# flexcompute/tidy3d

Hardware: AMD Instinct MI355X
Metric: Mcells/s on 512^3 Yee grid (higher is better)
Workload: dtype f32; 1 GPU; v0: vacuum, PEC walls, curl stencil only; 512^3 Yee cells, Ez point dipole (GaussianPulse 200 THz), random +-1e-3 initial fields; parallelism=z-slab x1, bytes_per_cell_step=72

## Files before the change

include/fdtd_hip.h:

```cpp
#ifndef FDTD_HIP_H
#define FDTD_HIP_H

#include <stddef.h>
#include <stdint.h>

#ifdef __cplusplus
extern "C" {
#endif

typedef struct FdtdSolver FdtdSolver;

enum { FDTD_BC_PEC = 0, FDTD_BC_PMC = 1, FDTD_BC_PERIODIC = 2, FDTD_BC_NEIGHBOR = 3 };
enum { FDTD_MON_TIME = 0, FDTD_MON_DFT = 1, FDTD_MON_FLUX_TIME = 2 ,
       FDTD_MON_TIME_SPARSE = 3 ,
       FDTD_MON_DFT_SPARSE = 4 ,
       FDTD_MON_DFT_LATTICE = 5  };
enum { FDTD_VARIANT_AUTO = 0, FDTD_VARIANT_SIMPLE = 1, FDTD_VARIANT_ZMARCH = 2, FDTD_VARIANT_FUSED = 3 };
enum { FDTD_FLAG_TIME_KERNELS = 1 };

typedef struct FdtdConfig {
  int32_t nx, ny, nz;
  int32_t bc[6];
  int32_t device;
  int32_t variant;
// ... 173 lines not shown
       FDTD_OPT_EDGE_ZCHUNK = 14,
       FDTD_OPT_GRAPH = 15,
       FDTD_OPT_TWOSTEP = 16,
       FDTD_OPT_SHELL_PAIRS = 17,
       FDTD_OPT_STRIP = 18,
       FDTD_OPT_SHELL2 = 19,
       FDTD_OPT_SHELL2_SHAPE = 20,
       FDTD_OPT_DEBUG_SYNC = 21,
       FDTD_OPT_TILE_SPLIT = 22,
       FDTD_OPT_DISP = 23,
       FDTD_OPT_SRC_PAGED = 25,
       FDTD_OPT_WHATIF = 24,
       FDTD_OPT_SLAB_BOXES_FIRST = 26,
       FDTD_OPT_SEAM_DEFER = 27,
       FDTD_OPT_AXIS_SHIFT = 28,
       FDTD_OPT_LDS_PAD = 10  };
int fdtd_set_option(FdtdSolver* h, int key, int value);
int fdtd_get_seam_stats(FdtdSolver* h, FdtdSeamStats* out);
int fdtd_reset(FdtdSolver* h);

#define FDTD_SWEEP_WORD(lb, opt, w) (((int64_t)(w) << 48) | ((int64_t)(lb) << 32) | (int64_t)(opt))
#define FDTD_SWEEP_WORD_OPT(word) ((int)((word) & 0xffffffff))
#define FDTD_SWEEP_WORD_LB(word) ((int)(((word) >> 32) & 0xffff))
#define FDTD_SWEEP_WORD_W(word) ((int)(((word) >> 48) & 0xff))
int fdtd_get_sweep_words(FdtdSolver* h, int64_t* out, int cap);
int fdtd_sweep_table(int64_t* out, int cap);

#ifdef __cplusplus
}
#endif
#endif
```

tidy3d_amd/csrc/fdtd_capi.hip:

```cpp
#include <hip/hip_runtime.h>
#include <rccl/rccl.h>

#include <array>
#include <cmath>
#include <cstdarg>
#include <cstdio>
#include <cstdlib>
#include <cstring>
#include <deque>
#include <map>
#include <string>
#include <utility>
#include <algorithm>
#include <vector>

#include "../../include/fdtd_hip.h"
#include "fdtd_kernels.hpp"
#include "fdtd_fused2.hpp"
#include "fdtd_strip.hpp"
#include "fdtd_shell2_host.hpp"
#include "fdtd_aniso.hpp"
#include "fdtd_modulation.hpp"
#include "fdtd_conformal.hpp"
#include "fdtd_near_field.hpp"
// ... 179 lines not shown
  std::string err;
  std::vector<DevBuf> bufs;
  float* fbase[6] = {};
  FieldP f{};
  float* fbase2[6] = {};
  FieldP f2{};
  float* fbase3[6] = {};
  FieldP f3{};
  float* step_base[2] = {};
  size_t field_bytes = 0;
  float *ip[3] = {}, *idl[3] = {};
  uint32_t* mat4 = nullptr;
  uint32_t* mat4b = nullptr;
  uint32_t* roww = nullptr;
  std::vector<uint32_t> roww_host;
  struct TileClasses { int W, zc; ClipP box; int nbx, nby, nbz; unsigned char* dev; long long n_bg, n_all; bool disp, src; };
  std::vector<TileClasses> tile_cls;
  int tile_split = -1;
  float2* lut = nullptr;
  int n_media = 0;
  float ca1 = 1.f, cb1 = 0.f;
  std::vector<float> cb_host;
  PmlAxisDev pml[3];
  float *damp_fb[3] = {}, *damp_fc[3] = {};
  int damp_lo[3] = {0, 0, 0}, damp_hi[3] = {0, 0, 0};
  bool has_damp = false;
  std::vector<AdeGroup> ade;
  Disp disp;
  SrcPaged spg;
  std::map<std::array<int, 6>, int> box_paged;
  int spg_on = -1;
  int whatif = 0;
// ... 787 lines not shown
    }
    tb.dump_floats = off;
    if (!boxes.empty()) {
      std::vector<int> ds((size_t)g.nz + 2, 0), dl;
      for (int k = 0; k <= g.nz; ++k) { ds[(size_t)k] = (int)dl.size(); if (k < g.nz) for (int b : per_plane[(size_t)k]) dl.push_back(b); }
      ds[(size_t)g.nz + 1] = (int)dl.size();
      if (dl.empty()) dl.push_back(0);
      if (dev_upload(h, &tb.dstart, (const int*)ds.data(), ds.size()) || dev_upload(h, &tb.dlist, (const int*)dl.data(), dl.size()) ||
          dev_upload(h, &tb.dboxes, (const DumpBox*)boxes.data(), boxes.size())) return nullptr;
    }
  }
  h->f2_tables.push_back(tb);
  return &h->f2_tables.back();
}

const FdtdSolver::TileClasses* tile_classes(FdtdSolver* h, int W, int zc, const ClipP& box, int nbx, int nby, int nbz, bool disp = false, bool src = false) {
  const bool mats = h->mat4 && !h->roww_host.empty();
  if ((!mats && !src) || h->tile_split == 0) return nullptr;
  for (const auto& t : h->tile_cls)
    if (t.W == W && t.zc == zc && t.nbx == nbx && t.nby == nby && t.nbz == nbz && t.box.j0 == box.j0 && t.box.j1 == box.j1 &&
        t.box.k0 == box.k0 && t.box.k1 == box.k1 && t.disp == disp && t.src == src) return &t;
  const GridP& g = h->g;
  const int R = W - 3, nbx_all = (g.nx + 255) / 256;
  std::vector<unsigned char> cls((size_t)nbx * nby * nbz, 0);
  long long n_bg = 0;
  for (int tz = 0; tz < nbz; ++tz)
    for (int tx = 0; tx < nbx; ++tx)
      for (int ty = 0; ty < nby; ++ty) {
        const int k0 = box.k0 + tz * zc, k1 = std::min(k0 + zc, box.k1);
        const int j0 = box.j0 + ty * R;
        unsigned char c = 0;
        for (int k = std::max(k0 - 1, 0); mats && k <= std::min(k1, g.nz - 1) && !c; ++k)
          for (int j = std::max(j0 - 2, 0); j <= std::min(j0 + R, g.ny - 1); ++j)
            if (h->roww_host[((size_t)k * g.ny + j) * nbx_all + tx] != kBgWord) { c = 1; break; }
        if (disp && c)
          for (int k = std::max(k0 - 1, 0); k <= std::min(k1, g.nz - 1) && c < 2; ++k)
            for (int j = std::max(j0 - 2, 0); j <= std::min(j0 + R, g.ny - 1); ++j)
              if (h->disp.dseg_host[((size_t)k * g.ny + j) * nbx_all + tx] >= 0) { c = 2; break; }
        n_bg += !c;
        if (src) {
          bool found = false;
          for (int k = std::max(k0 - 1, 0); k <= std::min(k1, g.nz - 1) && !found; ++k)
            for (int j = std::max(j0 - 2, 0); j <= std::min(j0 + R, g.ny - 1); ++j)
              if (h->spg.sseg_host[((size_t)k * g.ny + j) * nbx_all + tx] >= 0) { found = true; break; }
          if (found) c |= 4;
        }
        cls[((size_t)tz * nbx + tx) * nby + ty] = c;
      }
  FdtdSolver::TileClasses e{W, zc, box, nbx, nby, nbz, nullptr, n_bg, (long long)cls.size(), disp, src};
  if (dev_upload(h, &e.dev, (const unsigned char*)cls.data(), cls.size())) return nullptr;
  h->tile_cls.push_back(e);
  return &h->tile_cls.back();
}

void flush_seams(FdtdSolver* h, hipStream_t st);
int launch_fused2(FdtdSolver* h, long long n, hipStream_t st, const F2Table* tb, bool* sources2_done, bool* damp2_done = nullptr,
                  const ClipP* clip = nullptr, bool use_disp = false, bool e2_clip = false, const SrcP& sr = SrcP{}, bool defer_ok = false) {
  const bool inject = tb->with_sources;
  const GridP& g = h->g;
  if (use_disp && !h->mat4) return fail(h, "launch_fused2: dispersive cells in a pair without the materials grid");
  if (ensure_second_set(h)) return -1;
  int W = 16, zc = 32;
  const ClipP box = clip ? *clip : ClipP{0, g.nx, 0, g.ny, 0, g.nz};
  fused2_shape(h, &W, &zc, (clip && h->comm) ? clip : nullptr);
  if (clip && !h->comm && h->twostep_zc <= 0 && (long long)g.nx * g.ny * g.nz < (1LL << 28)) zc = std::min(zc, 16);
  zc = std::max(2, std::min(zc, box.k1 - box.k0));
  h->twostep_w_used = W; h->twostep_zc_used = zc;
// ... 60 lines not shown
      S.sseg_host.assign(nseg, -1);
      SrcT tab{};
      if (dev_upload(h, &S.sseg, (const int*)S.sseg_host.data(), nseg) || dev_upload(h, &S.tab, &tab, 1)) return -1;
    }
    if (S.sseg && S.state != 1) { sr_used.sseg = S.sseg; sr_used.t = S.tab; }
  }
  const int wv = h->whatif == 19 ? 9 : ((h->whatif >= 1 && h->whatif <= 15 && h->whatif != 9) ? h->whatif : 0);
  const auto word = [&](bool rep) {
    return fused2_opt(h->mem_hints != 0, h->mat4 != nullptr, !(tb->mons.empty() && (!tb->with_sources || h->src_h_nodes == 0) && !tb->dstart),
                      clip != nullptr, damp, use_disp, sr_used.sseg != nullptr, wv, rep, W);
  };
  const bool rep_capable = n_seams > 0 && !clip && (W == 16 || h->seam_defer == 2) && fused2_rep_word(word(false));
  const int opt = word(rep_capable && (h->seam_pending || h->whatif == 17));
  const auto no_sweep = [&] { return fail(h, "launch_fused2: no instantiation of the sweep for opt 0x%x, %d waves", opt, W); };
  if (!fused2_instantiated(fused2_lb(W, opt), opt)) return no_sweep();
  if (sr.sseg) { *sources2_done = true; h->spg.pairs++; }
  float* const rep_arr = h->seam_buf ? h->seam_buf + seam_scratch_floats(g, nbx) : nullptr;
  if (h->seam_pending && !rep_capable) flush_seams(h, st);
  h->seam_pending = false;
  bool defer = defer_ok && rep_capable && h->seam_defer != 0 && h->whatif == 0;
  if (defer) {
    bool e_post = false;
    for (const PointSrc& s : h->psrc) e_post = e_post || (s.n_e && n + 1 < s.n_steps);
    if ((e_post && !*sources2_done) || (h->has_damp && !dmp.e2)) defer = false;
  }
  const int blocks = remap ? ((total + 7) / 8) * 8 : total;
  const FdtdSolver::TileClasses* tc = tile_classes(h, W, zc, box, nbx, nby, nbz, use_disp, sr_used.sseg != nullptr);
  const bool split = tc && (use_disp || sr_used.sseg || (tc->n_bg > 0 && (h->tile_split == 1 || 8 * tc->n_bg >= tc->n_all)));
  const bool launched = launch_fused2_step(Fused2Launch{st, W, opt, blocks, g, h->f, h->f2, sp, mp, zc, nbx, nby, nbz, remap, inj, h->seam_buf, dmp, box,
                                                        TileClassP{split ? tc->dev : nullptr}, dp, sr_used});
  time_end(h, st);
  if (!launched) return no_sweep();
  {
    const int64_t word = FDTD_SWEEP_WORD(fused2_lb(W, opt), opt, W);
    if (std::find(h->sweep_words.begin(), h->sweep_words.end(), word) == h->sweep_words.end()) h->sweep_words.push_back(word);
  }
  if (n_seams > 0 && !(rep_capable && (h->whatif == 16 || h->whatif == 17))) {
    time_begin(h, 4, st);
    launch_seams(st, g, h->f2, sp, mp, h->seam_buf, n_seams, dmp, box, inj, sr, (defer || (h->whatif == 18 && rep_capable)) ? rep_arr : nullptr);
    time_end(h, st);
  }
  if (use_disp) h->disp.pairs++;
  if (!clip) swap_sets(h);
  if (defer) { h->seam_pending = true; h->seam_deferred_pairs++; }
  return 0;
// ... 1506 lines not shown
    return fail(nullptr, "fdtd_create: slab of %d x %d x %d cells exceeds the 2^32 cell index range", cfg->nx, cfg->ny, cfg->nz);
  for (int a = 0; a < 3; ++a) {
    const bool p0 = cfg->bc[2 * a] == FDTD_BC_PERIODIC, p1 = cfg->bc[2 * a + 1] == FDTD_BC_PERIODIC;
    if (p0 != p1 && a < 2) return fail(nullptr, "fdtd_create: periodic boundary must be set on both faces of axis %d", a);
    if (cfg->bc[2 * a + 1] == FDTD_BC_PMC) return fail(nullptr, "fdtd_create: PMC is supported on min faces only");
    if (a < 2 && (cfg->bc[2 * a] == FDTD_BC_NEIGHBOR || cfg->bc[2 * a + 1] == FDTD_BC_NEIGHBOR))
      return fail(nullptr, "fdtd_create: neighbour faces exist only along z");
  }
  int ndev = 0;
  if (hipGetDeviceCount(&ndev) != hipSuccess || ndev < 1) return fail(nullptr, "fdtd_create: no HIP device available");
  if (cfg->device < 0 || cfg->device >= ndev) return fail(nullptr, "fdtd_create: device %d out of range (%d devices)", cfg->device, ndev);
  FdtdSolver* h = new FdtdSolver();
  h->cfg = *cfg;
  h->no_jlo = getenv("FDTD_NO_JLO") != nullptr;
  if (hipSetDevice(cfg->device) != hipSuccess) { delete h; return fail(nullptr, "hipSetDevice(%d) failed", cfg->device); }
  GridP& g = h->g;
  g.nx = cfg->nx; g.ny = cfg->ny; g.nz = cfg->nz;
  g.sxy = (long long)cfg->nx * cfg->ny;
  g.bcx0 = cfg->bc[0]; g.bcx1 = cfg->bc[1]; g.bcy0 = cfg->bc[2]; g.bcy1 = cfg->bc[3];
  g.pec_z0 = cfg->bc[4] == FDTD_BC_PEC;
  g.psi_ghost = cfg->bc[4] == FDTD_BC_NEIGHBOR ? 1 : 0;
  g.ch = cfg->ch;
  h->zchunk = cfg->z_chunk > 0 ? cfg->z_chunk : 2;
  h->zchunk_f = cfg->z_chunk > 0 ? cfg->z_chunk : 16;
  h->user_geometry = cfg->z_chunk > 0;
  h->rows = 4;
  int rc = 0;
  const size_t fcount = (size_t)g.sxy * (g.nz + 2);
  h->field_bytes = fcount * sizeof(float);
  rc = alloc_field_set(h, h->fbase, fcount, 0);
// ... 889 lines not shown
    }
    case FDTD_OPT_PML_SPLIT: h->pml_split = value < 0 ? -1 : (value != 0); return 0;
    case FDTD_OPT_SHELL_PAIRS: h->shell_on = value < 0 ? -1 : value; return 0;
    case FDTD_OPT_STRIP: if (value % 64 < 1 || (value / 64 != 3 && value / 64 != 4)) break; h->strip_zc = value % 64; h->strip_occ = value / 64; return 0;
    case FDTD_OPT_SHELL2: h->shell2_on = value < 0 ? -1 : (value > 3 ? 1 : value); return 0;
    case FDTD_OPT_DEBUG_SYNC: h->debug_sync = value != 0; return 0;
    case FDTD_OPT_TILE_SPLIT: h->tile_split = value < 0 ? -1 : (value != 0); return 0;
    case FDTD_OPT_SRC_PAGED:
      h->spg_on = value < 0 ? -1 : (value != 0);
      if (h->spg.state == -1 && value != 0) h->spg.state = 0;
      return 0;
    case FDTD_OPT_SLAB_BOXES_FIRST: if (value < 0 || value > 3) break; h->slab_boxes_first = value; return 0;
    case FDTD_OPT_WHATIF: if (value < 0 || value > 19) break; h->whatif = value; return 0;
    case FDTD_OPT_SEAM_DEFER: if (value > 2) break; h->seam_defer = value < 0 ? -1 : value; return 0;
    case FDTD_OPT_AXIS_SHIFT: if (value < 0 || value > 2) break; h->axis_shift = value; return 0;
    case FDTD_OPT_DISP:
      if (h->disp.state == 1 && value == 0) break;
      h->disp_on = value < 0 ? -1 : (value != 0);
      if (h->disp.state == -1 && value != 0) h->disp.state = 0;
      return 0;
    case FDTD_OPT_SHELL2_SHAPE: {
      if (value <= 0) { h->shell2_qw = 0; h->shell2_ww = 8; h->shell2_zcw = 0; h->shell2_ws = 6; h->shell2_zcs = 0; return 0; }
      const int qw = value % 128, ww = (value >> 7) % 8 + ((value >> 7) % 8 == 0 ? 8 : 0), zcw = (value >> 10) % 128;
      const int ws = (value >> 17) % 16, zcs = (value >> 21) % 128;
      if ((qw != 0 && qw < 3) || qw > 64 || ws > 8) break;
      h->shell2_qw = qw; h->shell2_ww = ww; h->shell2_zcw = zcw;
      h->shell2_ws = ws > 0 ? ws : 6; h->shell2_zcs = zcs;
      return 0;
    }
    case FDTD_OPT_FUSED_LB: if (value != 0 && value != 256 && value != 512 && value != 1024) break; h->fused_lb = value; return 0;
// ... 27 lines not shown
  out->src_paged_pairs = (int32_t)std::min<long long>(h->spg.pairs, 0x7fffffff);
  out->struct_bytes = (int32_t)sizeof(FdtdStats);
  return 0;
}

int fdtd_get_seam_stats(FdtdSolver* h, FdtdSeamStats* out) {
  if (!h || !out) return -1;
  out->seam_deferred_pairs = h->seam_deferred_pairs;
  out->seam_flushes = h->seam_flushes;
  out->seam_pending = h->seam_pending ? 1 : 0;
  out->reserved = 0;
  out->seam_flush_ms = h->seam_flush_ms;
  return 0;
}

int fdtd_get_sweep_words(FdtdSolver* h, int64_t* out, int cap) {
  if (!h || (cap > 0 && !out)) return -1;
  const int n = (int)h->sweep_words.size();
  for (int i = 0; i < n && i < cap; ++i) out[i] = h->sweep_words[i];
  return n;
}

int fdtd_sweep_table(int64_t* out, int cap) {
  if (cap > 0 && !out) return -1;
  static const int64_t table[] = {
#define FDTD_F2_X(LBV, OV) FDTD_SWEEP_WORD(LBV, OV, 0),
      FDTD_F2_LIST_ALL(FDTD_F2_X)
#undef FDTD_F2_X
  };
  const int n = (int)(sizeof(table) / sizeof(table[0]));
// ... 6 lines not shown
```

tidy3d_amd/csrc/fdtd_fused2.hpp:

```cpp
#pragma once
#include "fdtd_kernels.hpp"

namespace fdtd {

constexpr int kMaxInj = 256;
struct InjP {
  int n;
  const int* start;
  const int4* ent;
  const float* val;
  const float* val2;
  int e2_in_sweep;
  float* cap;
  const int* dstart;
  const int* dlist;
  const struct DumpBox* dboxes;
  float* dump;
};
struct DumpBox {
  int lo0, lo1, lo2, nx, ny, nz;
  int off[6];
};
constexpr int kMaxDumps = 8;
struct DampT {
  const float* fb[3];
  const float* fc[3];
  int e2;
};
struct ClipP { int i0, i1, j0, j1, k0, k1; };
struct TileClassP { const unsigned char* cls; };
struct DispP {
  const int* dseg;
  const float* cs;
  float* e1;
};
struct SrcT {
  const float* e1;
  const float* h2;
  const float* e2;
  int use_h2, use_e2;
  const float* e1b;
  const float* h2b;
  const float* e2b;
};
struct SrcP {
  const int* sseg = nullptr;
  const SrcT* t = nullptr;
};
constexpr int kF2NT = 1;
constexpr int kF2Mat = 2;
constexpr int kF2Mon = 4;
constexpr int kF2Damp = 8;
constexpr int kF2Clip = 16;
constexpr int kF2Disp = 32;
constexpr int kF2Src = 64;
constexpr int kF2WhatifShift = 8, kF2WhatifMask = 15;
constexpr int kF2NoExj = 4096;
constexpr int kF2Rep = 8192;
constexpr int fused2_whatif(int opt) { return (opt >> kF2WhatifShift) & kF2WhatifMask; }
constexpr int fused2_whatif_word(int wv) { return kF2NT | (wv << kF2WhatifShift); }
constexpr bool fused2_rep_word(int opt) { return (opt & ~(kF2NT | kF2Mat | kF2Damp)) == 0; }

constexpr int fused2_opt(bool nt, bool mat, bool mon, bool clip, bool damp, bool disp, bool src, int whatif, bool rep, int W) {
  int opt = (nt ? kF2NT : 0) | (mat ? kF2Mat : 0) | (mon ? kF2Mon : 0) | (clip ? kF2Clip : (damp ? kF2Damp : 0)) |
            (disp ? kF2Disp | kF2NT : 0) | (src ? kF2Src | kF2Mon | kF2NT : 0);
  if (whatif && opt == kF2NT && (W == 16 || whatif == 13 || whatif == 14)) opt = fused2_whatif_word(whatif);
  return opt | (rep ? kF2Rep : 0);
}
constexpr int fused2_lb(int waves, int opt) {
  if ((opt & kF2Rep) || fused2_whatif(opt)) return 1024;
  if (waves <= 8) return 512;
  return (waves <= 12 && !(opt & (kF2Src | kF2Disp))) ? 768 : 1024;
}

#define FDTD_F2_AT512(X, O) X(512, (O))
#define FDTD_F2_AT768(X, O) X(768, (O))
// ... 68 lines not shown
  return fused2_lds_bytes(lb, opt, w) == ((size_t)(fused2_exj(lb, opt) ? 9 : 8) * w * 64 + ((opt & 8) ? 2 * 64 : 0)) * sizeof(float4) + ((opt & 2) ? (size_t)kMaxMedia * sizeof(float2) : 0);
}
#define FDTD_F2_X(LBV, OV) && fused2_lds_pinned(LBV, OV)
static_assert(true FDTD_F2_LIST_ALL(FDTD_F2_X), "fused2_lds_bytes: the LDS of a listed instantiation changed");
#undef FDTD_F2_X
constexpr int kMaxCap = 1024;
constexpr int kSeamArrays = 13;

void launch_inject_values(hipStream_t st, float* val, const float* w_re, const float* w_im, const float2* wave,
                          long long step, int n);
struct Fused2Launch {
  hipStream_t st;
  int waves, opt, grid_blocks;
  GridP g; FieldP a, b; StepP s; MatP m;
  int zchunk, nbx, nby, nbz, xcd_remap;
  InjP inj; float* seam; DampT dmp; ClipP clip; TileClassP tcl; DispP dp; SrcP sr;
};
#define FDTD_F2_ARGS(L) (L).g, (L).a, (L).b, (L).s, (L).m, (L).zchunk, (L).nbx, (L).nby, (L).nbz, (L).xcd_remap, (L).inj, (L).seam, (L).dmp, (L).clip, (L).tcl, (L).dp, (L).sr
#define FDTD_F2_CASE(LBV, OV)                                                                                                      \
  case fused2_key(LBV, OV):                                                                                                        \
    hipLaunchKernelGGL((fused2_step_kernel<LBV, OV>), dim3(L.grid_blocks, 1, 1), dim3(64, L.waves, 1), fused2_lds_bytes(LBV, OV, L.waves), L.st, \
                       FDTD_F2_ARGS(L));                                                                                           \
    return true;
#define FDTD_F2_LAUNCHER(NAME, LIST)                                                                                               \
  bool NAME(const Fused2Launch& L) {                                                                                               \
    switch (fused2_key(fused2_lb(L.waves, L.opt), L.opt)) { LIST(FDTD_F2_CASE) default: return false; }                            \
  }
bool launch_fused2_step(const Fused2Launch& L);
bool launch_fused2_step_src(const Fused2Launch& L);
bool launch_fused2_step_whatif(const Fused2Launch& L);
bool launch_fused2_step_disp(const Fused2Launch& L);
bool launch_fused2_step_clip(const Fused2Launch& L);
void launch_inject_table(hipStream_t st, float* tab, long long stride, long long off, const float* w_re, const float* w_im,
// ... 26 lines not shown
```

tidy3d_amd/csrc/fdtd_kernels2.hpp:

```cpp
#pragma once
#include "fdtd_fused2.hpp"

namespace fdtd {

__global__ __launch_bounds__(256) void pair_record_kernel(PairRecP r, GridP g, FieldP a, FieldP b, const float* cap) {
  const int mi = blockIdx.y / 6, ic = blockIdx.y % 6;
  if (mi >= r.n_mon || ic >= r.nc[mi]) return;
  const BoxP bx = r.box[mi];
  const long long cells = (long long)bx.nx * bx.ny * bx.nz;
  const long long t = (long long)blockIdx.x * blockDim.x + threadIdx.x;
  if (t >= cells) return;
  const int c = r.comp[mi][ic];
  const int lx = (int)(t % bx.nx), ly = (int)((t / bx.nx) % bx.ny), lz = (int)(t / ((long long)bx.nx * bx.ny));
  const long long p = (long long)(bx.lo2 + lz) * g.sxy + (long long)(bx.lo1 + ly) * g.nx + bx.lo0 + lx;
  const long long idx = (long long)ic * cells + t;
  const float* fa = c == 0 ? a.ex : (c == 1 ? a.ey : (c == 2 ? a.ez : (c == 3 ? a.hx : (c == 4 ? a.hy : a.hz))));
  const float* fb = c == 0 ? b.ex : (c == 1 ? b.ey : (c == 2 ? b.ez : (c == 3 ? b.hx : (c == 4 ? b.hy : b.hz))));
  const float mid = cap[r.cap_off[mi] + idx];
  float* on = r.out_n[mi];
  float* om = r.out_m[mi];
  if (c < 3) {
    if (on && !r.pre_done) on[idx] = 1.0f * fa[p];
    if (om) om[idx] = 1.0f * mid;
  } else {
// ... 93 lines not shown
  return v;
}

__device__ __forceinline__ int lane_value(int v, int l) {
#if defined(__HIP_DEVICE_COMPILE__)
  return __builtin_amdgcn_readlane(v, l);
#else
  return __shfl(v, l);
#endif
}

template <int LB, int OPT>
__device__ __forceinline__ void fused2_step_tile(const GridP& g, const FieldP& a, const FieldP& b, const StepP& s, const MatP& m,
                                                 int zchunk, int nbx, int nby, int nbz, const InjP& inj,
                                                 float* __restrict__ seam, const DampT& dmp, const ClipP& clip, int t,
                                                 const DispP& dp, const SrcP& sr) {
  constexpr int V = 4;
  constexpr bool SRC = (OPT & kF2Src) != 0;
  constexpr bool NT = (OPT & kF2NT) != 0, MAT = (OPT & kF2Mat) != 0, MON = (OPT & kF2Mon) != 0;
  constexpr bool DISP = (OPT & kF2Disp) != 0;
  constexpr int WHATIF = fused2_whatif(OPT);
  constexpr int PF = (WHATIF >= 10 && WHATIF <= 12) ? WHATIF : 0;
  constexpr bool EZL = WHATIF == 15;
  constexpr bool EXJ = (WHATIF == 0 && (OPT & kF2NoExj) == 0) || WHATIF == 13 || EZL;
  constexpr bool E1S = PF != 0 || EZL;
  constexpr int XE = E1S ? 6 : 8, XZ = 7;
  [[maybe_unused]] constexpr int NPF = PF == 11 ? 2 : (PF ? 3 : 0);
  constexpr int NXCH = E1S ? 6 : 8;
  static_assert((!PF && !EZL) || (OPT & 0xff & ~kF2NT) == 0, "prefetch instantiations: the vacuum sweep only");
  constexpr bool DAMP = (OPT & kF2Damp) != 0;
  constexpr bool CLIP = (OPT & kF2Clip) != 0;
  constexpr bool REP = (OPT & kF2Rep) != 0;
  static_assert(!REP || (!CLIP && !PF && !EZL && !DISP && !SRC), "deferred seam repair: plain, materials and absorber sweeps of the whole grid");
  const bool per_x = CLIP && g.bcx0 == BC_PERIODIC;
  const int tile_y = t % nby;
  const int tile_x = (t / nby) % nbx;
  const int tile_z = t / (nby * nbx);
  HIP_DYNAMIC_SHARED(float4, xch)
  const int tx = threadIdx.x;
  const int ty = __builtin_amdgcn_readfirstlane((int)threadIdx.y);
  const int W = blockDim.y, R = W - 3;
  const int slot = W * 64;
  const int me = ty * 64 + tx;
  {
    const float4 z4 = {0.f, 0.f, 0.f, 0.f};
#pragma unroll
    for (int q = 0; q < NXCH; ++q) xch[q * slot + me] = z4;
  }
  [[maybe_unused]] float4* xdm = xch + (EXJ ? 9 : 8) * slot;
  [[maybe_unused]] float2* lut_s = reinterpret_cast<float2*>(xdm + (DAMP ? 2 * 64 : 0));
  if constexpr (MAT) {
    for (int q = me; q < m.n_media; q += slot) lut_s[q] = m.lut[q];
  }
  if constexpr (DAMP) {
    if (ty == 0) {
      const int ii = (tile_x * 64 + tx) * V;
      float4 b4 = {1.f, 1.f, 1.f, 1.f}, c4 = {1.f, 1.f, 1.f, 1.f};
      if (ii < g.nx) { b4 = *reinterpret_cast<const float4*>(dmp.fb[0] + ii); c4 = *reinterpret_cast<const float4*>(dmp.fc[0] + ii); }
      xdm[tx] = b4; xdm[64 + tx] = c4;
    }
  }
  __syncthreads();
  const float ca = m.ca1, cb = m.cb1;
  const int k0 = (CLIP ? clip.k0 : 0) + tile_z * zchunk;
  const int k1 = min(k0 + zchunk, CLIP ? clip.k1 : g.nz);
  const int kA = k0 > 0 ? k0 - 1 : 0;
  int j = (CLIP ? clip.j0 : 0) + tile_y * R + ty - 2;
  const bool row_ok = (j >= 0) && (j < g.ny);
  if (!row_ok) {
    if constexpr (WHATIF != 6 && WHATIF != 7 && WHATIF != 8)
      for (int k = kA; k <= k1; ++k) { __syncthreads(); if constexpr (WHATIF != 2) __syncthreads(); }
    return;
  }
  const int i0 = (tile_x * 64 + tx) * V;
  const unsigned ux = (unsigned)i0;
  const unsigned ub = ux * 4u;
  const unsigned ubc = (i0 < g.nx) ? ub : 0u;
  const bool act = (i0 < g.nx);
  const bool do_e1 = ty >= 1;
  const bool do_h2 = ty >= 1 && ty <= W - 2;
// ... 758 lines not shown
    if constexpr (DAMP) { bz_m = bzk; cz_m = czk; }
    if constexpr (MAT) rw_m = rw;
    if constexpr (SRC) ss_m = ss;
    cur ^= 1;
  };
  if constexpr (PF != 0) pf_issue(kA);
  for (int k = kA; k <= k1; k += 2) {
    body(k, LA);
    if (k + 1 <= k1) body(k + 1, LB2);
  }
}

template <int LB, int OPT>
__device__ __forceinline__ void fused2_tile_by_class(const GridP& g, const FieldP& a, const FieldP& b, const StepP& s, const MatP& m,
                                                     int zchunk, int nbx, int nby, int nbz, const InjP& inj, float* __restrict__ seam,
                                                     const DampT& dmp, const ClipP& clip, int t, const DispP& dp, const SrcP& sr, const TileClassP& tcl) {
  if constexpr ((OPT & kF2Mat) != 0) {
    if (tcl.cls) {
      const int cl = tcl.cls[t] & 3;
      if (cl == 0) {
        fused2_step_tile<LB, (OPT & ~(kF2Mat | kF2Disp))>(g, a, b, s, m, zchunk, nbx, nby, nbz, inj, seam, dmp, clip, t, dp, sr);
        return;
      }
      if constexpr ((OPT & kF2Disp) != 0) {
        if (cl == 1) {
          fused2_step_tile<LB, (OPT & ~kF2Disp)>(g, a, b, s, m, zchunk, nbx, nby, nbz, inj, seam, dmp, clip, t, dp, sr);
          return;
        }
      }
    }
  }
  fused2_step_tile<LB, OPT>(g, a, b, s, m, zchunk, nbx, nby, nbz, inj, seam, dmp, clip, t, dp, sr);
}

template <int LB, int OPT>
__global__ __launch_bounds__(LB, (LB == 512 ? 4 : 1)) void fused2_step_kernel(GridP g, FieldP a, FieldP b, StepP s, MatP m,
                                                         int zchunk, int nbx, int nby, int nbz, int xcd_remap,
                                                         InjP inj, float* __restrict__ seam, DampT dmp, ClipP clip, TileClassP tcl, DispP dp, SrcP sr) {
  const int total = nbx * nby * nbz;
  int t = blockIdx.x;
  if (xcd_remap == 1) {
    const int per = (total + 7) >> 3;
    t = (t & 7) * per + (t >> 3);
    if (t >= total) return;
  } else if (xcd_remap > 1) {
    const int G = xcd_remap, full = total / (8 * G) * (8 * G);
    if (t < full) {
      const int x = t & 7, mloc = t >> 3;
      t = ((mloc / G) * 8 + x) * G + mloc % G;
    }
    if (t >= total) return;
  }
  constexpr int OPTK = OPT | (fused2_exj(LB, OPT) ? 0 : kF2NoExj);
  if constexpr ((OPT & kF2Src) != 0) {
    if (tcl.cls && !(tcl.cls[t] & 4)) {
      fused2_tile_by_class<LB, (OPTK & ~kF2Src)>(g, a, b, s, m, zchunk, nbx, nby, nbz, inj, seam, dmp, clip, t, dp, sr, tcl);
      return;
    }
  }
  fused2_tile_by_class<LB, OPTK>(g, a, b, s, m, zchunk, nbx, nby, nbz, inj, seam, dmp, clip, t, dp, sr, tcl);
}

__global__ __launch_bounds__(256) void seam_kernel(GridP g, FieldP b, StepP s, MatP m,
                                                   const float* __restrict__ seam, int n_seams, DampT dmp, ClipP clip, InjP inj, SrcP sr,
                                                   float* __restrict__ rep) {
  const long long t = (long long)blockIdx.x * blockDim.x + threadIdx.x;
  const int nj = clip.j1 - clip.j0;
  const long long per = (long long)nj * (clip.k1 - clip.k0);
  if (t >= per * n_seams) return;
  const int sm = (int)(t / per);
  const int k = clip.k0 + (int)((t % per) / nj), j = clip.j0 + (int)(t % nj);
  const bool wrap = g.bcx0 == BC_PERIODIC && sm == n_seams - 1;
  const int c = wrap ? g.nx : (sm + 1) * 256;
  const int cc = wrap ? 0 : c;
  const bool wl = c - 1 >= clip.i0 && c - 1 < clip.i1, wr = cc >= clip.i0 && cc < clip.i1;
// ... 110 lines not shown
```

tidy3d_amd/lib.py:

```python
from __future__ import annotations

import ctypes as C
import os
from typing import Optional

from .exceptions import SolverLibraryError

_HERE = os.path.dirname(os.path.abspath(__file__))
DEFAULT_LIB = os.path.join(_HERE, "libfdtd_hip.so")



def _prefer_hw_queues() -> None:
    os.environ.setdefault("GPU_MAX_HW_QUEUES", "8")


SYMBOLS = (
    "fdtd_last_error", "fdtd_device_count", "fdtd_create", "fdtd_destroy", "fdtd_set_steps",
    "fdtd_set_media", "fdtd_set_material", "fdtd_set_material16", "fdtd_set_pml", "fdtd_set_absorber", "fdtd_add_ade",
    "fdtd_add_point_source", "fdtd_add_tfsf", "fdtd_add_monitor", "fdtd_get_monitor",
    "fdtd_set_field", "fdtd_get_field", "fdtd_set_shutoff", "fdtd_comm_unique_id",
    "fdtd_comm_init", "fdtd_run", "fdtd_run_bloch", "fdtd_get_stats", "fdtd_reset", "fdtd_set_option",
    "fdtd_far_field", "fdtd_set_mirror_plus", "fdtd_add_aniso", "fdtd_add_aniso_bloch", "fdtd_get_seam_stats",
    "fdtd_get_sweep_words", "fdtd_sweep_table", "fdtd_add_flux_time_monitor", "fdtd_get_monitor_bytes",
    "fdtd_add_field_time_monitor", "fdtd_add_field_dft_monitor", "fdtd_add_lattice_dft_monitor", "fdtd_add_modulation",
    "fdtd_add_pec_conformal",
    "fdtd_near_field", "fdtd_near_field_chunks",
)

BC_PEC, BC_PMC, BC_PERIODIC, BC_NEIGHBOR = 0, 1, 2, 3
MON_TIME, MON_DFT, MON_FLUX_TIME, MON_TIME_SPARSE, MON_DFT_SPARSE, MON_DFT_LATTICE = 0, 1, 2, 3, 4, 5
VARIANT_AUTO, VARIANT_SIMPLE, VARIANT_ZMARCH, VARIANT_FUSED = 0, 1, 2, 3
FLAG_TIME_KERNELS = 1
OPT_FLAGS, OPT_VARIANT, OPT_ZCHUNK, OPT_ROWS, OPT_XCD_REMAP, OPT_FUSED_LB, OPT_PML_FUSED, OPT_BND_PLANES, OPT_AUTOTUNE, OPT_PML_SPLIT, OPT_LDS_PAD, OPT_MEM_HINTS, OPT_PLACEMENT_TRIES, OPT_TBLOCK, OPT_EDGE_ZCHUNK, OPT_GRAPH, OPT_TWOSTEP, OPT_SHELL_PAIRS, OPT_STRIP, OPT_SHELL2, OPT_SHELL2_SHAPE, OPT_DEBUG_SYNC, OPT_TILE_SPLIT, OPT_DISP, OPT_WHATIF, OPT_SRC_PAGED, OPT_SLAB_BOXES_FIRST, OPT_SEAM_DEFER, OPT_AXIS_SHIFT = 0, 1, 2, 3, 4, 5, 6, 7, 8, 9, 10, 11, 12, 13, 14, 15, 16, 17, 18, 19, 20, 21, 22, 23, 24, 25, 26, 27, 28
F2_OFF_REASONS = {0: "", 1: "switched off", 2: "grid too small", 3: "z-slab rank", 4: "CPML (shell pairs not possible)",
                  5: "dispersive media not confined to a few planes along z", 6: "TFSF box while it injects", 7: "Bloch / PMC-plus faces (or rows not a multiple of 4 cells)", 8: "magnetic sources with absorber layers",
                  9: "magnetic source node on a tile seam", 10: "too many source nodes", 11: "two-pass kernels",
                  12: "CPML shell too large a part of the grid", 13: "no device memory for the third field set", 14: "wide material table (more than 1023 media)",
                  15: "time-modulated media", 16: "PEC-conformal boundaries"}


class FdtdConfig(C.Structure):
    _fields_ = [("nx", C.c_int32), ("ny", C.c_int32), ("nz", C.c_int32),
                ("bc", C.c_int32 * 6), ("device", C.c_int32), ("variant", C.c_int32),
                ("flags", C.c_int32), ("z_chunk", C.c_int32), ("ch", C.c_float),
                ("reserved", C.c_int32 * 6)]


class FdtdStats(C.Structure):
# ... 38 lines not shown
            raise SolverLibraryError(f"cannot load the HIP solver library '{path}': {e}") from e
        missing = [s for s in SYMBOLS if not hasattr(self.dll, s)]
        if missing:
            raise SolverLibraryError(f"'{path}' does not export: {', '.join(missing)}")
        d = self.dll
        vp, i32, i64, f32 = C.c_void_p, C.c_int32, C.c_int64, C.c_float
        d.fdtd_last_error.restype = C.c_char_p
        d.fdtd_last_error.argtypes = [vp]
        d.fdtd_device_count.restype = C.c_int
        d.fdtd_create.argtypes = [C.POINTER(FdtdConfig), C.POINTER(vp)]
        d.fdtd_destroy.argtypes = [vp]
        d.fdtd_destroy.restype = None
        d.fdtd_get_seam_stats.argtypes = [vp, C.POINTER(FdtdSeamStats)]
        d.fdtd_get_sweep_words.argtypes = [vp, C.POINTER(C.c_int64), C.c_int]
        d.fdtd_sweep_table.argtypes = [C.POINTER(C.c_int64), C.c_int]
        d.fdtd_set_steps.argtypes = [vp, C.c_int, vp, vp, C.c_int]
        d.fdtd_set_media.argtypes = [vp, vp, vp, C.c_int]
        d.fdtd_set_material.argtypes = [vp, vp, C.c_size_t]
        d.fdtd_set_material16.argtypes = [vp, vp, C.c_size_t]
        d.fdtd_set_pml.argtypes = [vp, C.c_int, C.c_int, C.c_int, vp, vp, vp, vp, vp, vp, C.c_int]
        d.fdtd_set_absorber.argtypes = [vp, C.c_int, C.c_int, C.c_int, vp, vp, C.c_int]
        d.fdtd_set_mirror_plus.argtypes = [vp, C.c_int, C.c_int]
        d.fdtd_add_ade.argtypes = [vp, C.c_int, i64, vp, C.c_int, vp, vp, f32]
        d.fdtd_add_aniso.argtypes = [vp, C.c_int, i64, vp, vp, vp, vp]
        d.fdtd_add_aniso_bloch.argtypes = [vp, C.c_int, i64, vp, vp, vp, vp, vp]
        d.fdtd_add_modulation.argtypes = [vp, C.c_int, i64, vp, vp, vp, vp, vp, vp, C.c_double, C.c_double]
        d.fdtd_add_pec_conformal.argtypes = [vp, C.c_int, i64, vp, vp, vp]
        d.fdtd_add_point_source.argtypes = [vp, i64, vp, vp, vp, vp, i64, vp, vp]
        d.fdtd_add_tfsf.argtypes = [vp, C.c_int, vp, vp, vp, vp, C.c_int, i64, vp,
                                    i64, vp, vp, vp, vp, i64, vp, vp, vp, vp]
# ... 95 lines not shown
```

Baseline: 204,700 Mcells/s.

## Add table-driven z-chunk plans for fused sweep workgroups with CU-balanced option

```diff
diff --git a/include/fdtd_hip.h b/include/fdtd_hip.h
--- a/include/fdtd_hip.h
+++ b/include/fdtd_hip.h
@@ -211,9 +211,11 @@
        FDTD_OPT_SLAB_BOXES_FIRST = 26,
        FDTD_OPT_SEAM_DEFER = 27,
        FDTD_OPT_AXIS_SHIFT = 28,
+       FDTD_OPT_CHUNK_PLAN = 29,
        FDTD_OPT_LDS_PAD = 10  };
 int fdtd_set_option(FdtdSolver* h, int key, int value);
 int fdtd_get_seam_stats(FdtdSolver* h, FdtdSeamStats* out);
+int fdtd_chunk_plan(int nx, int ny, int nz, int waves, int zc, int n_cu, int force, int32_t* out, int cap);
 int fdtd_reset(FdtdSolver* h);
 
 #define FDTD_SWEEP_WORD(lb, opt, w) (((int64_t)(w) << 48) | ((int64_t)(lb) << 32) | (int64_t)(opt))
diff --git a/tidy3d_amd/csrc/fdtd_capi.hip b/tidy3d_amd/csrc/fdtd_capi.hip
--- a/tidy3d_amd/csrc/fdtd_capi.hip
+++ b/tidy3d_amd/csrc/fdtd_capi.hip
@@ -217,8 +217,12 @@
   uint32_t* mat4b = nullptr;
   uint32_t* roww = nullptr;
   std::vector<uint32_t> roww_host;
-  struct TileClasses { int W, zc; ClipP box; int nbx, nby, nbz; unsigned char* dev; long long n_bg, n_all; bool disp, src; };
+  struct TileClasses { int W, zc; ClipP box; int nbx, nby, nbz; unsigned char* dev; long long n_bg, n_all; bool disp, src; int plan_id; };
   std::vector<TileClasses> tile_cls;
+  struct ChunkPlan { int W, zc, force, id; std::vector<int4> rec; int4* dev; };
+  std::deque<ChunkPlan> chunk_plans;
+  int chunk_plan = -1;
+  int n_cu = 256;
   int tile_split = -1;
   float2* lut = nullptr;
   int n_media = 0;
@@ -1036,43 +1040,56 @@
   return &h->f2_tables.back();
 }
 
-const FdtdSolver::TileClasses* tile_classes(FdtdSolver* h, int W, int zc, const ClipP& box, int nbx, int nby, int nbz, bool disp = false, bool src = false) {
+const FdtdSolver::TileClasses* tile_classes(FdtdSolver* h, int W, int zc, const ClipP& box, int nbx, int nby, int nbz, bool disp = false, bool src = false,
+                                            const FdtdSolver::ChunkPlan* plan = nullptr) {
   const bool mats = h->mat4 && !h->roww_host.empty();
   if ((!mats && !src) || h->tile_split == 0) return nullptr;
   for (const auto& t : h->tile_cls)
     if (t.W == W && t.zc == zc && t.nbx == nbx && t.nby == nby && t.nbz == nbz && t.box.j0 == box.j0 && t.box.j1 == box.j1 &&
-        t.box.k0 == box.k0 && t.box.k1 == box.k1 && t.disp == disp && t.src == src) return &t;
+        t.box.k0 == box.k0 && t.box.k1 == box.k1 && t.disp == disp && t.src == src && t.plan_id == (plan ? plan->id : 0)) return &t;
   const GridP& g = h->g;
   const int R = W - 3, nbx_all = (g.nx + 255) / 256;
-  std::vector<unsigned char> cls((size_t)nbx * nby * nbz, 0);
+  const size_t n_wg = plan ? plan->rec.size() : (size_t)nbx * nby * nbz;
+  std::vector<unsigned char> cls(n_wg, 0);
   long long n_bg = 0;
-  for (int tz = 0; tz < nbz; ++tz)
-    for (int tx = 0; tx < nbx; ++tx)
-      for (int ty = 0; ty < nby; ++ty) {
-        const int k0 = box.k0 + tz * zc, k1 = std::min(k0 + zc, box.k1);
-        const int j0 = box.j0 + ty * R;
-        unsigned char c = 0;
-        for (int k = std::max(k0 - 1, 0); mats && k <= std::min(k1, g.nz - 1) && !c; ++k)
-          for (int j = std::max(j0 - 2, 0); j <= std::min(j0 + R, g.ny - 1); ++j)
-            if (h->roww_host[((size_t)k * g.ny + j) * nbx_all + tx] != kBgWord) { c = 1; break; }
-        if (disp && c)
-          for (int k = std::max(k0 - 1, 0); k <= std::min(k1, g.nz - 1) && c < 2; ++k)
-            for (int j = std::max(j0 - 2, 0); j <= std::min(j0 + R, g.ny - 1); ++j)
-              if (h->disp.dseg_host[((size_t)k * g.ny + j) * nbx_all + tx] >= 0) { c = 2; break; }
-        n_bg += !c;
-        if (src) {
-          bool found = false;
-          for (int k = std::max(k0 - 1, 0); k <= std::min(k1, g.nz - 1) && !found; ++k)
-            for (int j = std::max(j0 - 2, 0); j <= std::min(j0 + R, g.ny - 1); ++j)
-              if (h->spg.sseg_host[((size_t)k * g.ny + j) * nbx_all + tx] >= 0) { found = true; break; }
-          if (found) c |= 4;
-        }
-        cls[((size_t)tz * nbx + tx) * nby + ty] = c;
-      }
-  FdtdSolver::TileClasses e{W, zc, box, nbx, nby, nbz, nullptr, n_bg, (long long)cls.size(), disp, src};
+  for (size_t t = 0; t < n_wg; ++t) {
+    const int tz = (int)(t / ((size_t)nbx * nby)), tx = plan ? plan->rec[t].x : (int)(t / nby) % nbx, ty = plan ? plan->rec[t].y : (int)(t % nby);
+    const int k0 = plan ? plan->rec[t].z : box.k0 + tz * zc, k1 = plan ? plan->rec[t].w : std::min(k0 + zc, box.k1);
+    const int j0 = box.j0 + ty * R;
+    unsigned char c = 0;
+    for (int k = std::max(k0 - 1, 0); mats && k <= std::min(k1, g.nz - 1) && !c; ++k)
+      for (int j = std::max(j0 - 2, 0); j <= std::min(j0 + R, g.ny - 1); ++j)
+        if (h->roww_host[((size_t)k * g.ny + j) * nbx_all + tx] != kBgWord) { c = 1; break; }
+    if (disp && c)
+      for (int k = std::max(k0 - 1, 0); k <= std::min(k1, g.nz - 1) && c < 2; ++k)
+        for (int j = std::max(j0 - 2, 0); j <= std::min(j0 + R, g.ny - 1); ++j)
+          if (h->disp.dseg_host[((size_t)k * g.ny + j) * nbx_all + tx] >= 0) { c = 2; break; }
+    n_bg += !c;
+    if (src) {
+      bool found = false;
+      for (int k = std::max(k0 - 1, 0); k <= std::min(k1, g.nz - 1) && !found; ++k)
+        for (int j = std::max(j0 - 2, 0); j <= std::min(j0 + R, g.ny - 1); ++j)
+          if (h->spg.sseg_host[((size_t)k * g.ny + j) * nbx_all + tx] >= 0) { found = true; break; }
+      if (found) c |= 4;
+    }
+    cls[t] = c;
+  }
+  FdtdSolver::TileClasses e{W, zc, box, nbx, nby, nbz, nullptr, n_bg, (long long)cls.size(), disp, src, plan ? plan->id : 0};
   if (dev_upload(h, &e.dev, (const unsigned char*)cls.data(), cls.size())) return nullptr;
   h->tile_cls.push_back(e);
   return &h->tile_cls.back();
+}
+
+constexpr bool chunk_plan_default(int ) { return false; }
+const FdtdSolver::ChunkPlan* chunk_plan(FdtdSolver* h, int W, int zc, int nbx, int nby, int mode) {
+  for (const auto& p : h->chunk_plans)
+    if (p.W == W && p.zc == zc && p.force == mode) return &p;
+  const GridP& g = h->g;
+  FdtdSolver::ChunkPlan p{W, zc, mode, (int)h->chunk_plans.size() + 1, {}, nullptr};
+  p.rec = mode == 0 ? fused2_uniform_plan(nbx, nby, g.nz, zc) : fused2_chunk_plan(nbx, nby, g.ny, W, g.nz, zc, h->n_cu, mode >= 2 ? mode : 0);
+  if (dev_upload(h, &p.dev, (const int4*)p.rec.data(), p.rec.size())) return nullptr;
+  h->chunk_plans.push_back(std::move(p));
+  return &h->chunk_plans.back();
 }
 
 void flush_seams(FdtdSolver* h, hipStream_t st);
@@ -1163,6 +1180,11 @@
   const int opt = word(rep_capable && (h->seam_pending || h->whatif == 17));
   const auto no_sweep = [&] { return fail(h, "launch_fused2: no instantiation of the sweep for opt 0x%x, %d waves", opt, W); };
   if (!fused2_instantiated(fused2_lb(W, opt), opt)) return no_sweep();
+  const FdtdSolver::ChunkPlan* plan = nullptr;
+  if (fused2_plan_word(opt)) {
+    plan = chunk_plan(h, W, zc, nbx, nby, h->chunk_plan < 0 ? (chunk_plan_default(opt) ? 1 : 0) : h->chunk_plan);
+    if (!plan) return -1;
+  }
   if (sr.sseg) { *sources2_done = true; h->spg.pairs++; }
   float* const rep_arr = h->seam_buf ? h->seam_buf + seam_scratch_floats(g, nbx) : nullptr;
   if (h->seam_pending && !rep_capable) flush_seams(h, st);
@@ -1173,11 +1195,13 @@
     for (const PointSrc& s : h->psrc) e_post = e_post || (s.n_e && n + 1 < s.n_steps);
     if ((e_post && !*sources2_done) || (h->has_damp && !dmp.e2)) defer = false;
   }
-  const int blocks = remap ? ((total + 7) / 8) * 8 : total;
-  const FdtdSolver::TileClasses* tc = tile_classes(h, W, zc, box, nbx, nby, nbz, use_disp, sr_used.sseg != nullptr);
+  const int n_wg = plan ? (int)plan->rec.size() : total;
+  const int blocks = remap ? ((n_wg + 7) / 8) * 8 : n_wg;
+  const FdtdSolver::TileClasses* tc = tile_classes(h, W, zc, box, nbx, nby, nbz, use_disp, sr_used.sseg != nullptr, plan);
   const bool split = tc && (use_disp || sr_used.sseg || (tc->n_bg > 0 && (h->tile_split == 1 || 8 * tc->n_bg >= tc->n_all)));
   const bool launched = launch_fused2_step(Fused2Launch{st, W, opt, blocks, g, h->f, h->f2, sp, mp, zc, nbx, nby, nbz, remap, inj, h->seam_buf, dmp, box,
-                                                        TileClassP{split ? tc->dev : nullptr}, dp, sr_used});
+                                                        TileClassP{split ? tc->dev : nullptr}, dp, sr_used,
+                                                        ChunkPlanP{plan ? plan->dev : nullptr, n_wg}});
   time_end(h, st);
   if (!launched) return no_sweep();
   {
@@ -2714,6 +2738,9 @@
   h->cfg = *cfg;
   h->no_jlo = getenv("FDTD_NO_JLO") != nullptr;
   if (hipSetDevice(cfg->device) != hipSuccess) { delete h; return fail(nullptr, "hipSetDevice(%d) failed", cfg->device); }
+#if defined(__HIPCC__)
+  { int cus = 0; if (hipDeviceGetAttribute(&cus, hipDeviceAttributeMultiprocessorCount, cfg->device) == hipSuccess && cus > 0) h->n_cu = cus; }
+#endif
   GridP& g = h->g;
   g.nx = cfg->nx; g.ny = cfg->ny; g.nz = cfg->nz;
   g.sxy = (long long)cfg->nx * cfg->ny;
@@ -3633,6 +3660,7 @@
     case FDTD_OPT_WHATIF: if (value < 0 || value > 19) break; h->whatif = value; return 0;
     case FDTD_OPT_SEAM_DEFER: if (value > 2) break; h->seam_defer = value < 0 ? -1 : value; return 0;
     case FDTD_OPT_AXIS_SHIFT: if (value < 0 || value > 2) break; h->axis_shift = value; return 0;
+    case FDTD_OPT_CHUNK_PLAN: if (value > 4096) break; h->chunk_plan = value < 0 ? -1 : value; return 0;
     case FDTD_OPT_DISP:
       if (h->disp.state == 1 && value == 0) break;
       h->disp_on = value < 0 ? -1 : (value != 0);
@@ -3690,6 +3718,14 @@
   return 0;
 }
 
+int fdtd_chunk_plan(int nx, int ny, int nz, int waves, int zc, int n_cu, int force, int32_t* out, int cap) {
+  if (nx < 1 || ny < 1 || nz < 1 || waves < 4 || waves > 16 || zc < 1 || n_cu < 1 || force < 0 || (cap > 0 && !out)) return -1;
+  const int R = waves - 3;
+  const std::vector<int4> rec = fused2_chunk_plan((nx + 255) / 256, (ny + R - 1) / R, ny, waves, nz, zc, n_cu, force);
+  for (size_t i = 0; i < rec.size() && (int)i < cap; ++i) { out[4 * i] = rec[i].x; out[4 * i + 1] = rec[i].y; out[4 * i + 2] = rec[i].z; out[4 * i + 3] = rec[i].w; }
+  return (int)rec.size();
+}
+
 int fdtd_get_sweep_words(FdtdSolver* h, int64_t* out, int cap) {
   if (!h || (cap > 0 && !out)) return -1;
   const int n = (int)h->sweep_words.size();
diff --git a/tidy3d_amd/csrc/fdtd_fused2.hpp b/tidy3d_amd/csrc/fdtd_fused2.hpp
--- a/tidy3d_amd/csrc/fdtd_fused2.hpp
+++ b/tidy3d_amd/csrc/fdtd_fused2.hpp
@@ -1,4 +1,6 @@
 #pragma once
+#include <algorithm>
+#include <vector>
 #include "fdtd_kernels.hpp"
 
 namespace fdtd {
@@ -29,6 +31,7 @@
 };
 struct ClipP { int i0, i1, j0, j1, k0, k1; };
 struct TileClassP { const unsigned char* cls; };
+struct ChunkPlanP { const int4* rec; int n; };
 struct DispP {
   const int* dseg;
   const float* cs;
@@ -56,10 +59,62 @@
 constexpr int kF2Src = 64;
 constexpr int kF2WhatifShift = 8, kF2WhatifMask = 15;
 constexpr int kF2NoExj = 4096;
+constexpr int kF2NoPlan = 16384;
 constexpr int kF2Rep = 8192;
 constexpr int fused2_whatif(int opt) { return (opt >> kF2WhatifShift) & kF2WhatifMask; }
 constexpr int fused2_whatif_word(int wv) { return kF2NT | (wv << kF2WhatifShift); }
 constexpr bool fused2_rep_word(int opt) { return (opt & ~(kF2NT | kF2Mat | kF2Damp)) == 0; }
+
+inline std::vector<int4> fused2_chunk_plan(int nbx, int nby, int ny, int W, int nz, int zc, int n_cu, int force) {
+  const int R = W - 3, rows_last = ny - (nby - 1) * R;
+  const bool ragged = nby > 1 && rows_last < R;
+  const int cf = ragged ? nbx * (nby - 1) : nbx * nby, cr = ragged ? nbx : 0;
+  const auto n_ragged = [&](int n) { return std::min(nz, std::max(1, (2 * n * (rows_last + 3) + W - 1) / (2 * W))); };
+  const auto count = [&](int n) { return (long long)cf * n + (long long)cr * n_ragged(n); };
+  int n = std::min(std::max(force, 1), nz), more_f = 0, more_r = 0;
+  if (force <= 0) {
+    const long long uniform = count(std::min(nz, (nz + zc - 1) / zc));
+    long long target = uniform / n_cu * n_cu;
+    if (target < 2LL * n_cu || target < cf + cr) target = uniform;
+    n = 1;
+    while (n < nz && count(n + 1) <= target) ++n;
+    if (n < nz) {
+      const long long more = std::max(0LL, target - count(n));
+      more_f = (int)std::min<long long>(more, cf);
+      more_r = n_ragged(n) < nz ? (int)std::min<long long>(more - more_f, cr) : 0;
+    }
+  }
+  std::vector<int4> rec;
+  rec.reserve((size_t)count(n) + more_f + more_r);
+  int seen_f = 0, seen_r = 0;
+  for (int tx = 0; tx < nbx; ++tx)
+    for (int ty = 0; ty < nby; ++ty) {
+      const bool last = ragged && ty == nby - 1;
+      const int m = last ? n_ragged(n) + (seen_r++ < more_r ? 1 : 0) : n + (seen_f++ < more_f ? 1 : 0);
+      for (int c = 0, k0 = 0; c < m; ++c) {
+        const int len = nz / m + (c < nz % m ? 1 : 0);
+        rec.push_back(int4{tx, ty, k0, k0 + len});
+        k0 += len;
+      }
+    }
+  std::stable_sort(rec.begin(), rec.end(), [](const int4& a, const int4& b) {
+    const int la = a.w - a.z, lb = b.w - b.z;
+    if (la != lb) return la > lb;
+    if (a.z != b.z) return a.z < b.z;
+    return a.x != b.x ? a.x < b.x : a.y < b.y;
+  });
+  return rec;
+}
+constexpr bool fused2_plan_word(int opt) {
+  return (opt & kF2Clip) == 0 && opt != (kF2Disp | kF2Mat | kF2NT | kF2Damp) && opt != (kF2Src | kF2Mon | kF2NT | kF2Mat);
+}
+inline std::vector<int4> fused2_uniform_plan(int nbx, int nby, int nz, int zc) {
+  std::vector<int4> rec;
+  for (int k0 = 0; k0 < nz; k0 += zc)
+    for (int tx = 0; tx < nbx; ++tx)
+      for (int ty = 0; ty < nby; ++ty) rec.push_back(int4{tx, ty, k0, std::min(k0 + zc, nz)});
+  return rec;
+}
 
 constexpr int fused2_opt(bool nt, bool mat, bool mon, bool clip, bool damp, bool disp, bool src, int whatif, bool rep, int W) {
   int opt = (nt ? kF2NT : 0) | (mat ? kF2Mat : 0) | (mon ? kF2Mon : 0) | (clip ? kF2Clip : (damp ? kF2Damp : 0)) |
@@ -158,9 +213,9 @@
   int waves, opt, grid_blocks;
   GridP g; FieldP a, b; StepP s; MatP m;
   int zchunk, nbx, nby, nbz, xcd_remap;
-  InjP inj; float* seam; DampT dmp; ClipP clip; TileClassP tcl; DispP dp; SrcP sr;
-};
-#define FDTD_F2_ARGS(L) (L).g, (L).a, (L).b, (L).s, (L).m, (L).zchunk, (L).nbx, (L).nby, (L).nbz, (L).xcd_remap, (L).inj, (L).seam, (L).dmp, (L).clip, (L).tcl, (L).dp, (L).sr
+  InjP inj; float* seam; DampT dmp; ClipP clip; TileClassP tcl; DispP dp; SrcP sr; ChunkPlanP plan;
+};
+#define FDTD_F2_ARGS(L) (L).g, (L).a, (L).b, (L).s, (L).m, (L).zchunk, (L).nbx, (L).nby, (L).nbz, (L).xcd_remap, (L).inj, (L).seam, (L).dmp, (L).clip, (L).tcl, (L).dp, (L).sr, (L).plan
 #define FDTD_F2_CASE(LBV, OV)                                                                                                      \
   case fused2_key(LBV, OV):                                                                                                        \
     hipLaunchKernelGGL((fused2_step_kernel<LBV, OV>), dim3(L.grid_blocks, 1, 1), dim3(64, L.waves, 1), fused2_lds_bytes(LBV, OV, L.waves), L.st, \
diff --git a/tidy3d_amd/csrc/fdtd_kernels2.hpp b/tidy3d_amd/csrc/fdtd_kernels2.hpp
--- a/tidy3d_amd/csrc/fdtd_kernels2.hpp
+++ b/tidy3d_amd/csrc/fdtd_kernels2.hpp
@@ -131,7 +131,7 @@
 __device__ __forceinline__ void fused2_step_tile(const GridP& g, const FieldP& a, const FieldP& b, const StepP& s, const MatP& m,
                                                  int zchunk, int nbx, int nby, int nbz, const InjP& inj,
                                                  float* __restrict__ seam, const DampT& dmp, const ClipP& clip, int t,
-                                                 const DispP& dp, const SrcP& sr) {
+                                                 const DispP& dp, const SrcP& sr, const ChunkPlanP& plan) {
   constexpr int V = 4;
   constexpr bool SRC = (OPT & kF2Src) != 0;
   constexpr bool NT = (OPT & kF2NT) != 0, MAT = (OPT & kF2Mat) != 0, MON = (OPT & kF2Mon) != 0;
@@ -150,9 +150,15 @@
   constexpr bool REP = (OPT & kF2Rep) != 0;
   static_assert(!REP || (!CLIP && !PF && !EZL && !DISP && !SRC), "deferred seam repair: plain, materials and absorber sweeps of the whole grid");
   const bool per_x = CLIP && g.bcx0 == BC_PERIODIC;
-  const int tile_y = t % nby;
-  const int tile_x = (t / nby) % nbx;
-  const int tile_z = t / (nby * nbx);
+  int tile_y, tile_x, pk0, pk1;
+  if constexpr ((OPT & (kF2Clip | kF2NoPlan)) == 0) {
+    const int4 r = plan.rec[t];
+    tile_x = r.x; tile_y = r.y; pk0 = r.z; pk1 = r.w;
+  } else {
+    tile_y = t % nby; tile_x = (t / nby) % nbx;
+    pk0 = clip.k0 + t / (nby * nbx) * zchunk;
+    pk1 = min(pk0 + zchunk, clip.k1);
+  }
   HIP_DYNAMIC_SHARED(float4, xch)
   const int tx = threadIdx.x;
   const int ty = __builtin_amdgcn_readfirstlane((int)threadIdx.y);
@@ -179,8 +185,7 @@
   }
   __syncthreads();
   const float ca = m.ca1, cb = m.cb1;
-  const int k0 = (CLIP ? clip.k0 : 0) + tile_z * zchunk;
-  const int k1 = min(k0 + zchunk, CLIP ? clip.k1 : g.nz);
+  const int k0 = pk0, k1 = pk1;
   const int kA = k0 > 0 ? k0 - 1 : 0;
   int j = (CLIP ? clip.j0 : 0) + tile_y * R + ty - 2;
   const bool row_ok = (j >= 0) && (j < g.ny);
@@ -969,30 +974,30 @@
 template <int LB, int OPT>
 __device__ __forceinline__ void fused2_tile_by_class(const GridP& g, const FieldP& a, const FieldP& b, const StepP& s, const MatP& m,
                                                      int zchunk, int nbx, int nby, int nbz, const InjP& inj, float* __restrict__ seam,
-                                                     const DampT& dmp, const ClipP& clip, int t, const DispP& dp, const SrcP& sr, const TileClassP& tcl) {
+                                                     const DampT& dmp, const ClipP& clip, int t, const DispP& dp, const SrcP& sr, const TileClassP& tcl, const ChunkPlanP& plan) {
   if constexpr ((OPT & kF2Mat) != 0) {
     if (tcl.cls) {
       const int cl = tcl.cls[t] & 3;
       if (cl == 0) {
-        fused2_step_tile<LB, (OPT & ~(kF2Mat | kF2Disp))>(g, a, b, s, m, zchunk, nbx, nby, nbz, inj, seam, dmp, clip, t, dp, sr);
+        fused2_step_tile<LB, (OPT & ~(kF2Mat | kF2Disp))>(g, a, b, s, m, zchunk, nbx, nby, nbz, inj, seam, dmp, clip, t, dp, sr, plan);
         return;
       }
       if constexpr ((OPT & kF2Disp) != 0) {
         if (cl == 1) {
-          fused2_step_tile<LB, (OPT & ~kF2Disp)>(g, a, b, s, m, zchunk, nbx, nby, nbz, inj, seam, dmp, clip, t, dp, sr);
+          fused2_step_tile<LB, (OPT & ~kF2Disp)>(g, a, b, s, m, zchunk, nbx, nby, nbz, inj, seam, dmp, clip, t, dp, sr, plan);
           return;
         }
       }
     }
   }
-  fused2_step_tile<LB, OPT>(g, a, b, s, m, zchunk, nbx, nby, nbz, inj, seam, dmp, clip, t, dp, sr);
+  fused2_step_tile<LB, OPT>(g, a, b, s, m, zchunk, nbx, nby, nbz, inj, seam, dmp, clip, t, dp, sr, plan);
 }
 
 template <int LB, int OPT>
 __global__ __launch_bounds__(LB, (LB == 512 ? 4 : 1)) void fused2_step_kernel(GridP g, FieldP a, FieldP b, StepP s, MatP m,
                                                          int zchunk, int nbx, int nby, int nbz, int xcd_remap,
-                                                         InjP inj, float* __restrict__ seam, DampT dmp, ClipP clip, TileClassP tcl, DispP dp, SrcP sr) {
-  const int total = nbx * nby * nbz;
+                                                         InjP inj, float* __restrict__ seam, DampT dmp, ClipP clip, TileClassP tcl, DispP dp, SrcP sr, ChunkPlanP plan) {
+  const int total = fused2_plan_word(OPT) ? plan.n : nbx * nby * nbz;
   int t = blockIdx.x;
   if (xcd_remap == 1) {
     const int per = (total + 7) >> 3;
@@ -1006,14 +1011,14 @@
     }
     if (t >= total) return;
   }
-  constexpr int OPTK = OPT | (fused2_exj(LB, OPT) ? 0 : kF2NoExj);
+  constexpr int OPTK = OPT | (fused2_exj(LB, OPT) ? 0 : kF2NoExj) | (fused2_plan_word(OPT) ? 0 : kF2NoPlan);
   if constexpr ((OPT & kF2Src) != 0) {
     if (tcl.cls && !(tcl.cls[t] & 4)) {
-      fused2_tile_by_class<LB, (OPTK & ~kF2Src)>(g, a, b, s, m, zchunk, nbx, nby, nbz, inj, seam, dmp, clip, t, dp, sr, tcl);
+      fused2_tile_by_class<LB, (OPTK & ~kF2Src)>(g, a, b, s, m, zchunk, nbx, nby, nbz, inj, seam, dmp, clip, t, dp, sr, tcl, plan);
       return;
     }
   }
-  fused2_tile_by_class<LB, OPTK>(g, a, b, s, m, zchunk, nbx, nby, nbz, inj, seam, dmp, clip, t, dp, sr, tcl);
+  fused2_tile_by_class<LB, OPTK>(g, a, b, s, m, zchunk, nbx, nby, nbz, inj, seam, dmp, clip, t, dp, sr, tcl, plan);
 }
 
 __global__ __launch_bounds__(256) void seam_kernel(GridP g, FieldP b, StepP s, MatP m,
diff --git a/tidy3d_amd/lib.py b/tidy3d_amd/lib.py
--- a/tidy3d_amd/lib.py
+++ b/tidy3d_amd/lib.py
@@ -25,14 +25,14 @@
     "fdtd_get_sweep_words", "fdtd_sweep_table", "fdtd_add_flux_time_monitor", "fdtd_get_monitor_bytes",
     "fdtd_add_field_time_monitor", "fdtd_add_field_dft_monitor", "fdtd_add_lattice_dft_monitor", "fdtd_add_modulation",
     "fdtd_add_pec_conformal",
-    "fdtd_near_field", "fdtd_near_field_chunks",
+    "fdtd_near_field", "fdtd_near_field_chunks", "fdtd_chunk_plan",
 )
 
 BC_PEC, BC_PMC, BC_PERIODIC, BC_NEIGHBOR = 0, 1, 2, 3
 MON_TIME, MON_DFT, MON_FLUX_TIME, MON_TIME_SPARSE, MON_DFT_SPARSE, MON_DFT_LATTICE = 0, 1, 2, 3, 4, 5
 VARIANT_AUTO, VARIANT_SIMPLE, VARIANT_ZMARCH, VARIANT_FUSED = 0, 1, 2, 3
 FLAG_TIME_KERNELS = 1
-OPT_FLAGS, OPT_VARIANT, OPT_ZCHUNK, OPT_ROWS, OPT_XCD_REMAP, OPT_FUSED_LB, OPT_PML_FUSED, OPT_BND_PLANES, OPT_AUTOTUNE, OPT_PML_SPLIT, OPT_LDS_PAD, OPT_MEM_HINTS, OPT_PLACEMENT_TRIES, OPT_TBLOCK, OPT_EDGE_ZCHUNK, OPT_GRAPH, OPT_TWOSTEP, OPT_SHELL_PAIRS, OPT_STRIP, OPT_SHELL2, OPT_SHELL2_SHAPE, OPT_DEBUG_SYNC, OPT_TILE_SPLIT, OPT_DISP, OPT_WHATIF, OPT_SRC_PAGED, OPT_SLAB_BOXES_FIRST, OPT_SEAM_DEFER, OPT_AXIS_SHIFT = 0, 1, 2, 3, 4, 5, 6, 7, 8, 9, 10, 11, 12, 13, 14, 15, 16, 17, 18, 19, 20, 21, 22, 23, 24, 25, 26, 27, 28
+OPT_FLAGS, OPT_VARIANT, OPT_ZCHUNK, OPT_ROWS, OPT_XCD_REMAP, OPT_FUSED_LB, OPT_PML_FUSED, OPT_BND_PLANES, OPT_AUTOTUNE, OPT_PML_SPLIT, OPT_LDS_PAD, OPT_MEM_HINTS, OPT_PLACEMENT_TRIES, OPT_TBLOCK, OPT_EDGE_ZCHUNK, OPT_GRAPH, OPT_TWOSTEP, OPT_SHELL_PAIRS, OPT_STRIP, OPT_SHELL2, OPT_SHELL2_SHAPE, OPT_DEBUG_SYNC, OPT_TILE_SPLIT, OPT_DISP, OPT_WHATIF, OPT_SRC_PAGED, OPT_SLAB_BOXES_FIRST, OPT_SEAM_DEFER, OPT_AXIS_SHIFT, OPT_CHUNK_PLAN = 0, 1, 2, 3, 4, 5, 6, 7, 8, 9, 10, 11, 12, 13, 14, 15, 16, 17, 18, 19, 20, 21, 22, 23, 24, 25, 26, 27, 28, 29
 F2_OFF_REASONS = {0: "", 1: "switched off", 2: "grid too small", 3: "z-slab rank", 4: "CPML (shell pairs not possible)",
                   5: "dispersive media not confined to a few planes along z", 6: "TFSF box while it injects", 7: "Bloch / PMC-plus faces (or rows not a multiple of 4 cells)", 8: "magnetic sources with absorber layers",
                   9: "magnetic source node on a tile seam", 10: "too many source nodes", 11: "two-pass kernels",
@@ -101,6 +101,7 @@
         d.fdtd_get_seam_stats.argtypes = [vp, C.POINTER(FdtdSeamStats)]
         d.fdtd_get_sweep_words.argtypes = [vp, C.POINTER(C.c_int64), C.c_int]
         d.fdtd_sweep_table.argtypes = [C.POINTER(C.c_int64), C.c_int]
+        d.fdtd_chunk_plan.argtypes = [C.c_int] * 7 + [C.POINTER(C.c_int32), C.c_int]
         d.fdtd_set_steps.argtypes = [vp, C.c_int, vp, vp, C.c_int]
         d.fdtd_set_media.argtypes = [vp, vp, vp, C.c_int]
         d.fdtd_set_material.argtypes = [vp, vp, C.c_size_t]
```

Result: no change. 205,200 Mcells/s, median of 2 (+0.2%).
